# kai-neumann/OrthoSfM

Measured on AMD Instinct MI355X. Metric: image-pairs matched/sec + BA iterations/sec (N images, M tracks) at 1/2/4/8 GPU, higher is better.
Workload: dtype i8; 1 GPU; 50 orthographic images, 20000 SIFT features/img, exhaustive matching (1225 pairs, low-res gate + two-way + cross-check + lists; SURVEY 8d's unit of work: up to, not including, RANSAC-F -- the pass through RANSAC-F is `with_geometric_verification`); views=50, features_per_view=20000, pairs=1225

## Files before the change

### orthosfm_amd/csrc/match_api.hip

```cpp
#include <algorithm>
#include <atomic>
#include <cfloat>
#include <cmath>
#include <cstring>
#include <chrono>
#include <condition_variable>
#include <deque>
#include <functional>
#include <mutex>
#include <queue>
#include <thread>
#include <vector>

#include "match_kernels.h"
#include "cashash_kernels.h"
#include <random>
#include "osfm_common.h"
#include "ransac_kernels.h"

namespace osfm {

static thread_local std::string g_last_error;

void set_error(const char *fmt, ...)
{
    char buf[1024];
    va_list ap;
    va_start(ap, fmt);
    vsnprintf(buf, sizeof(buf), fmt, ap);
    va_end(ap);
    g_last_error = buf;
}

namespace {

inline int round_up(int x, int m) { return (x + m - 1) / m * m; }

struct ViewData {
    bool set = false;
    int ns = 0, nu = 0;
    int ns_pad = 0, nu_pad = 0;
    DeviceBuffer sift, sift_corr, surf, surf_corr;
    DeviceBuffer sift_raw, sift_raw_corr, special, special_corr, special_map, special_slot;
    int n_special = 0;
    int surf_norm2_max = 0;
    DeviceBuffer cas_hash[2], cas_bucket[2], cas_start[2], cas_items[2], cas_rec[2];
    DeviceBuffer positions;
    int n_positions = -1;
    hipEvent_t ready = nullptr;
    ~ViewData() { event_destroy(ready); }
    ViewData() = default;
    ViewData(const ViewData &) = delete;
    ViewData &operator=(const ViewData &) = delete;
};

void build_lowe_table(float lowe, bool is_signed, std::vector<int32_t> *tab)
{
    const volatile float sq = lowe * lowe;
    const float sq_lowe = sq;
    const int dmax = is_signed ? 32258 : 65534;
    tab->assign(32768, 0x7fffffff);
    for (int d2 = 0; d2 <= dmax; d2 += 2) {
        int lo = 0, hi = dmax / 2 + 1;
        while (lo < hi) {
            const int mid = (lo + hi) / 2;
            const float ratio = static_cast<float>(2 * mid) / static_cast<float>(d2);
            if (ratio > sq_lowe) hi = mid; else lo = mid + 1;
        }
        (*tab)[d2 / 2] = lo > dmax / 2 ? 0x7fffffff : 2 * lo;
    }
}

int max_d1_for(float dist_thres, bool is_signed)
{
    const volatile float sq = dist_thres * dist_thres;
    const float sq_dist = sq;
    const int dmax = is_signed ? 32258 : 65534;
    int best = -1;
    int lo = 0, hi = dmax;
    if (!(static_cast<float>(0) > sq_dist)) {
        while (lo < hi) {
            const int mid = (lo + hi + 1) / 2;
            if (static_cast<float>(mid) > sq_dist) hi = mid - 1; else lo = mid;
        }
        best = lo;
    }
    return best;
}

}
}

using namespace osfm;

struct osfm_matcher {
    int device = 0;
    hipStream_t stream = nullptr;
    osfm_match_options opts;
    std::vector<ViewData> views;
    DeviceBuffer lowe_sift, lowe_surf;
    LoweTable tab_sift, tab_surf;
    std::mutex mu;
    hipStream_t up_stream = nullptr;
    std::mutex up_mu;

    DeviceBuffer d_problems[2], rowparts, colparts, out, keep, mark_off[2], counts[2];
    DeviceBuffer exact_items, exact_count, stage_in, flags;
    DeviceBuffer sp_parts, sp_col, d_spjobs;
    DeviceBuffer clock_probe;
    DeviceBuffer zero_tile;
    int special_max = 512;
    int expect_pairs = 0;
    DeviceBuffer d_m12_off, d_len12, d_corr_off, d_keep_pair, d_corr;
    DeviceBuffer d_corr_alt;
    hipStream_t copy_stream = nullptr;
    hipEvent_t ev_compact[2] = {nullptr, nullptr}, ev_copied[2] = {nullptr, nullptr};
    bool copied_used[2] = {false, false};
    DeviceBuffer d_jobs, d_inl, d_inl_count, d_corr2, d_gather_off;
    hipEvent_t ev[2][2] = {{nullptr, nullptr}, {nullptr, nullptr}};
    hipEvent_t ev_sp[2] = {nullptr, nullptr};
    char *pin_ptr[2] = {nullptr, nullptr};
    size_t pin_bytes[2] = {0, 0};
    hipEvent_t pin_ev[2] = {nullptr, nullptr};
    bool pin_used[2] = {false, false};
    unsigned pin_next = 0;

    DeviceBuffer cas_proj[2], cas_sum[2], cas_avg[2], cas_state;
    std::atomic<bool> cas_dirty{true};

    osfm_match_stats stats;

    struct Staging { int32_t *ptr = nullptr; size_t ints = 0; int users = 0; };
    struct PairRequest {
        int kind;
        int v1, v2, num_features;
        int32_t *m12, *m21, *len12, *len21, *count;
        int status = OSFM_OK;
        bool done = false;
        std::string error;
        Staging *stage = nullptr;
        int64_t src12 = 0, src21 = 0;
        int32_t n12 = 0, n21 = 0;
    };
    std::vector<Staging *> comb_staging;

    std::vector<osfm_matcher *> shards;
    std::vector<Staging> shard_stage;
    std::atomic<unsigned> next_shard{0};
    std::mutex multi_mu;
    std::mutex comb_mu;
    std::condition_variable comb_cv;
    std::deque<PairRequest *> comb_queue;
    bool comb_leader = false;
};

namespace {

struct PairPlan {
    int v1, v2;
    int ns1, nu1, ns2, nu2;
    bool has_sift, has_surf;
    int64_t off12, off21;
    int len12, len21;
    int prob_index[2];
};

struct BatchResult {
    std::vector<PairPlan> plans;
    std::vector<int32_t> counts;
    int64_t out_ints = 0;
};

int check_view(const osfm_matcher *m, int v, const char *what)
{
    if (v < 0 || v >= (int)m->views.size()) {
        set_error("%s: view id %d out of range [0, %zu)", what, v, m->views.size());
        return OSFM_E_ARG;
    }
    if (!m->views[v].set) {
        set_error("%s: view %d has not been set", what, v);
        return OSFM_E_STATE;
    }
    return OSFM_OK;
}

struct BatchMode {
    int limit = 0;
    bool lowres = false;
    bool apply = true;
    int type_mask = 3;
    int expect = 0;
};

int ensure_cashash(osfm_matcher *m);

int run_batch(osfm_matcher *m, const osfm_pair *pairs, int num_pairs, const BatchMode &mode,
    BatchResult *res)
{
    const int lowres_limit = mode.limit;
    const bool cascade = m->opts.matcher_type == OSFM_MATCHER_CASCADE_HASHING && mode.limit == 0;
    if (cascade) OSFM_RETURN_IF(ensure_cashash(m));
    res->plans.assign(num_pairs, PairPlan());
    res->counts.assign(num_pairs, 0);
    std::vector<MatchProblem> probs[2];
    std::vector<SpecialJob> spjobs, spjobs_wide;
    struct SpEntry { int problem, side, view, units, nchunk; };
    std::vector<SpEntry> spentries;
    int64_t sp_recs = 0, sp_cols = 0;
    std::vector<int64_t> mark_off[2];
    int64_t out_ints = 0, rowpart_recs = 0, colpart_recs = 0, keep_bytes = 0, total_queries = 0;
    int total_blocks[2] = {0, 0}, max_n[2] = {0, 0};
    bool needs_mask[2] = {false, false};
    bool any_special[2] = {false, false};
    bool any_c0[2] = {false, false}, any_corrected[2] = {false, false};
    int64_t macs = 0, alg_bytes = 0, macs_surf = 0;
    int64_t cas_queries[2] = {0, 0};

    int64_t rb_estimate = 0;
    for (int p = 0; p < num_pairs; ++p) {
        const int v1 = pairs[p].view_1;
        if (v1 >= 0 && v1 < (int)m->views.size())
            rb_estimate += (std::max(m->views[v1].ns, m->views[v1].nu) + kRowsPerBlock - 1) / kRowsPerBlock;
    }
    static const int forced_seg_tiles = [] { const char *e = getenv("OSFM_SEG_TILES"); return e ? atoi(e) : 0; }();
    auto choose_seg_cols = [&](int n2) {
        const int ncyc = (n2 + kCycleCols - 1) / kCycleCols;
        int cyc;
        if (forced_seg_tiles > 0) cyc = std::max(1, forced_seg_tiles / 16);
        else {
            constexpr int64_t kWantBlocks = 2048;
            const int64_t want = (kWantBlocks + std::max<int64_t>(rb_estimate, 1) - 1) / std::max<int64_t>(rb_estimate, 1);
            const int nseg = (int)std::min<int64_t>(std::max<int64_t>(want, 1), ncyc);
            cyc = (ncyc + nseg - 1) / nseg;
        }
        cyc = std::min(cyc, kSegColsMax / kCycleCols);
        return cyc * kCycleCols;
    };

    for (int p = 0; p < num_pairs; ++p) {
        PairPlan &pl = res->plans[p];
        pl.v1 = pairs[p].view_1; pl.v2 = pairs[p].view_2;
        OSFM_RETURN_IF(check_view(m, pl.v1, "match"));
        OSFM_RETURN_IF(check_view(m, pl.v2, "match"));
        const ViewData &a = m->views[pl.v1], &b = m->views[pl.v2];
        pl.ns1 = a.ns; pl.nu1 = a.nu; pl.ns2 = b.ns; pl.nu2 = b.nu;
        pl.has_sift = a.ns > 0 && (mode.type_mask & 1);
        pl.has_surf = a.nu > 0 && (mode.type_mask & 2);
        if (cascade && !m->opts.cascade_keep_empty_blocks) {
            if (b.ns == 0) pl.has_sift = false;
            if (b.nu == 0) pl.has_surf = false;
        }
        if (mode.lowres && pl.has_sift) pl.has_surf = false;
        if (lowres_limit > 0) {
            pl.ns1 = std::min(pl.ns1, lowres_limit); pl.ns2 = std::min(pl.ns2, lowres_limit);
            pl.nu1 = std::min(pl.nu1, lowres_limit); pl.nu2 = std::min(pl.nu2, lowres_limit);
        }
        const int e1 = pl.has_sift ? pl.ns1 : 0;
        const int e2 = pl.has_sift ? pl.ns2 : 0;
        pl.len12 = e1 + (pl.has_surf ? pl.nu1 : 0);
        pl.len21 = e2 + (pl.has_surf ? pl.nu2 : 0);
        pl.off12 = out_ints; out_ints += round_up(pl.len12, 4);
        pl.off21 = out_ints; out_ints += round_up(pl.len21, 4);
        pl.prob_index[0] = pl.prob_index[1] = -1;
        for (int type = 0; type < 2; ++type) {
            if (type == 0 ? !pl.has_sift : !pl.has_surf) continue;
            MatchProblem pr;
            memset(&pr, 0, sizeof(pr));
            pr.n1 = type == 0 ? pl.ns1 : pl.nu1;
            pr.n2 = type == 0 ? pl.ns2 : pl.nu2;
            pr.A = (type == 0 ? a.sift : a.surf).as<int8_t>();
            pr.B = (type == 0 ? b.sift : b.surf).as<int8_t>();
            pr.corrA = (type == 0 ? a.sift_corr : a.surf_corr).as<int32_t>();
            pr.corrB = (type == 0 ? b.sift_corr : b.surf_corr).as<int32_t>();
            pr.A_raw = (type == 0 ? a.sift_raw : a.surf).as<int8_t>();
            pr.corrA_raw = (type == 0 ? a.sift_raw_corr : a.surf_corr).as<int32_t>();
            const bool limited = lowres_limit > 0;
            const int n_special = (type == 0 && !limited) ? a.n_special : 0;
            pr.n_special = n_special;
            pr.A_special = a.special.as<int8_t>();
            pr.corrA_special = a.special_corr.as<int32_t>();
            pr.special_map = a.special_map.as<int32_t>();
            pr.special_slot = n_special > 0 ? a.special_slot.as<int32_t>() : nullptr;
            const bool empty = pr.n1 == 0 || pr.n2 == 0;
            if (limited) needs_mask[type] = true;
            pr.B_raw = (type == 0 ? b.sift_raw : b.surf).as<int8_t>();
            pr.c0 = (type == 1 || b.n_special == 0) ? 1 : 0;
            if (type == 0 && !limited && !cascade && !empty && (a.n_special > 0 || b.n_special > 0) &&
                a.n_special <= m->special_max && b.n_special <= m->special_max) {
                pr.sp = 1; pr.c0 = 1;
                pr.nsA = a.n_special; pr.nsB = b.n_special;
                pr.n_special = 0;
                pr.special_slot = a.n_special > 0 ? a.special_slot.as<int32_t>() : nullptr;
                pr.B_special = b.special.as<int8_t>();
                pr.corrB_special = b.special_corr.as<int32_t>();
                pr.special_map_B = b.special_map.as<int32_t>();
                pr.special_slot_B = b.n_special > 0 ? b.special_slot.as<int32_t>() : nullptr;
                for (int side = 0; side < 2; ++side) {
                    const int ns = side == 0 ? pr.nsA : pr.nsB, no = side == 0 ? pr.n2 : pr.n1;
                    if (ns == 0) continue;
                    const int units = (ns + 31) / 32;
                    pr.sp_wide[side] = units > kSpSlots ? 1 : 0;
                    const int chunk_cols = pr.sp_wide[side] ? kSpWideChunk : kSpChunk;
                    const int nchunk = (no + chunk_cols - 1) / chunk_cols;
                    pr.sp_row_off[side] = sp_recs; sp_recs += (int64_t)nchunk * round_up(ns, 32);
                    pr.sp_col_off[side] = sp_cols; sp_cols += round_up(no, 32);
                    spentries.push_back({(int)probs[type].size(), side, side == 0 ? pl.v2 : pl.v1, units, nchunk});
                }
            }
            if (!empty && !limited) (pr.c0 ? any_c0 : any_corrected)[type] = true;
            if (!empty && pr.n_special > 0) any_special[type] = true;
            pr.nrb_main = empty ? 0 : (pr.n1 + kRowsPerBlock - 1) / kRowsPerBlock;
            pr.nrb = pr.nrb_main + (empty ? 0 : (pr.n_special + kRowsPerBlock - 1) / kRowsPerBlock);
            pr.seg_cols = (pr.c0 && !limited && pr.n_special == 0 && !empty) ? choose_seg_cols(pr.n2) : kSegCols;
            pr.nseg = empty ? 0 : (pr.n2 + pr.seg_cols - 1) / pr.seg_cols;
            pr.n2stride = round_up(pr.n2, kCycleCols);
            pr.block_start = total_blocks[type];
            if (cascade) {
                const ViewData *vd[2] = {&a, &b};
                for (int side = 0; side < 2; ++side) {
                    pr.cas_rec[side] = vd[side]->cas_rec[type].ptr;
                    pr.cas_start[side] = vd[side]->cas_start[type].as<int32_t>();
                    pr.cas_items[side] = vd[side]->cas_items[type].as<int32_t>();
                }
                pr.cas_state_off[0] = cas_queries[type]; cas_queries[type] += pr.n1;
                pr.cas_state_off[1] = cas_queries[type]; cas_queries[type] += pr.n2;
            } else {
                total_blocks[type] += pr.nrb * pr.nseg;
                pr.rowpart_off = rowpart_recs;
                rowpart_recs += (int64_t)pr.nseg * pr.nrb * kRowsPerBlock;
                pr.colpart_off = colpart_recs;
                colpart_recs += (int64_t)pr.nrb * pr.n2stride;
            }
            pr.m12 = reinterpret_cast<int32_t *>(pl.off12 + (type == 0 ? 0 : e1));
            pr.m21 = reinterpret_cast<int32_t *>(pl.off21 + (type == 0 ? 0 : e2));
            pr.out_off12 = (type == 1 && mode.apply) ? e2 : 0;
            pr.out_off21 = (type == 1 && mode.apply) ? e1 : 0;
            if (type == 1) {
                const long long bound = (long long)a.surf_norm2_max * (long long)b.surf_norm2_max;
                pr.force_exact = bound > 32767LL * 32767LL ? 1 : 0;
            }
            pl.prob_index[type] = (int)probs[type].size();
            mark_off[type].push_back(keep_bytes); keep_bytes += round_up(pr.n1, 16);
            mark_off[type].push_back(keep_bytes); keep_bytes += round_up(pr.n2, 16);
            max_n[type] = std::max(max_n[type], std::max(pr.n1, pr.n2));
            total_queries += pr.n1 + pr.n2;
            probs[type].push_back(pr);
            if (!empty) {
                const int dim = type == 0 ? 128 : 64;
                macs += (int64_t)pr.n1 * pr.n2 * dim;
                if (type == 1) macs_surf += (int64_t)pr.n1 * pr.n2 * dim;
                alg_bytes += (int64_t)(pr.n1 + pr.n2) * (dim + 4);
            }
        }
    }
    res->out_ints = out_ints;

    double grow = 1.0;
    if (mode.expect > num_pairs && num_pairs > 0) grow = 1.02 * (double)mode.expect / num_pairs;
    auto grown = [&](int64_t n) { return (size_t)((double)std::max<int64_t>(n, 1) * std::max(grow, 1.0)); };
    OSFM_RETURN_IF(m->out.reserve(grown(std::max<int64_t>(out_ints, 4)) * 4));
    OSFM_RETURN_IF(m->rowparts.reserve(grown(rowpart_recs) * sizeof(RowPart)));
    OSFM_RETURN_IF(m->colparts.reserve(grown(colpart_recs) * sizeof(ColPart)));
    OSFM_RETURN_IF(m->keep.reserve(grown(std::max<int64_t>(keep_bytes, 16))));
    OSFM_RETURN_IF(m->exact_items.reserve(grown(total_queries) * sizeof(ExactItem)));
    OSFM_RETURN_IF(m->exact_count.reserve(16));
    OSFM_RETURN_IF(m->sp_parts.reserve((size_t)std::max<int64_t>(sp_recs, 1) * sizeof(RowPart)));
    hipStream_t s = m->stream;
    {
        std::vector<uint8_t> seen(m->views.size(), 0);
        for (int p = 0; p < num_pairs; ++p)
            for (int v : {res->plans[p].v1, res->plans[p].v2})
                if (!seen[v]) { seen[v] = 1; if (m->views[v].ready) OSFM_HIP_CHECK(hipStreamWaitEvent(s, m->views[v].ready, 0)); }
    }
    std::stable_sort(spentries.begin(), spentries.end(), [](const SpEntry &x, const SpEntry &y) {
        return x.view != y.view ? x.view < y.view : x.units < y.units;
    });
    for (size_t e = 0; e < spentries.size();) {
        SpecialJob j;
        memset(&j, 0, sizeof(j));
        const SpEntry &f = spentries[e];
        if (f.units > kSpSlots) {
            j.problem[0] = f.problem; j.side[0] = f.side; j.count = 0;
            for (int c = 0; c < f.nchunk; ++c) { j.chunk = c; spjobs_wide.push_back(j); }
            ++e;
            continue;
        }
        if (f.units > 1) {
            j.problem[0] = f.problem; j.side[0] = f.side; j.count = 0;
            ++e;
        } else {
            int c = 0;
            while (c < kSpSlots && e < spentries.size() && spentries[e].view == f.view && spentries[e].units == 1) {
                j.problem[c] = spentries[e].problem; j.side[c] = spentries[e].side; ++c; ++e;
            }
            j.count = c;
        }
        for (int c = 0; c < f.nchunk; ++c) { j.chunk = c; spjobs.push_back(j); }
    }
    OSFM_RETURN_IF(m->sp_col.reserve((size_t)std::max<int64_t>(sp_cols, 1) * 4));
    OSFM_RETURN_IF(m->d_spjobs.reserve(std::max<size_t>(spjobs.size() + spjobs_wide.size(), 1) * sizeof(SpecialJob)));
    if (!spjobs.empty())
        OSFM_HIP_CHECK(hipMemcpyAsync(m->d_spjobs.ptr, spjobs.data(), spjobs.size() * sizeof(SpecialJob),
            hipMemcpyHostToDevice, s));
    if (!spjobs_wide.empty())
        OSFM_HIP_CHECK(hipMemcpyAsync(m->d_spjobs.as<SpecialJob>() + spjobs.size(), spjobs_wide.data(),
            spjobs_wide.size() * sizeof(SpecialJob), hipMemcpyHostToDevice, s));
    int32_t *d_out = m->out.as<int32_t>();
    OSFM_HIP_CHECK(hipMemsetAsync(d_out, 0xff, (size_t)std::max<int64_t>(out_ints, 4) * 4, s));

    OSFM_HIP_CHECK(hipMemsetAsync(m->exact_count.ptr, 0, 16, s));
    bool timed[2] = {false, false};
    bool probed = false;
    for (int type = 0; type < 2; ++type) {
        const int np = (int)probs[type].size();
        if (np == 0) continue;
        for (auto &pr : probs[type]) {
            pr.m12 = d_out + reinterpret_cast<intptr_t>(pr.m12);
            pr.m21 = d_out + reinterpret_cast<intptr_t>(pr.m21);
        }
        OSFM_RETURN_IF(m->d_problems[type].reserve(np * sizeof(MatchProblem)));
        OSFM_RETURN_IF(m->mark_off[type].reserve(np * 2 * sizeof(int64_t)));
        OSFM_RETURN_IF(m->counts[type].reserve(np * sizeof(int32_t)));
        OSFM_HIP_CHECK(hipMemcpyAsync(m->d_problems[type].ptr, probs[type].data(),
            np * sizeof(MatchProblem), hipMemcpyHostToDevice, s));
        OSFM_HIP_CHECK(hipMemcpyAsync(m->mark_off[type].ptr, mark_off[type].data(),
            np * 2 * sizeof(int64_t), hipMemcpyHostToDevice, s));
        OSFM_HIP_CHECK(hipMemsetAsync(m->counts[type].ptr, 0, np * sizeof(int32_t), s));
        const MatchProblem *dp = m->d_problems[type].as<MatchProblem>();
        const LoweTable tab = type == 0 ? m->tab_sift : m->tab_surf;
        const int ecap = (int)std::min<int64_t>(total_queries, 0x7fffffff);
        int32_t *ecount = m->exact_count.as<int32_t>() + type;

        if (cascade) {
            OSFM_HIP_CHECK(hipEventRecord(m->ev[type][0], s));
            timed[type] = true;
            OSFM_RETURN_IF(m->cas_state.reserve((size_t)std::max<int64_t>(cas_queries[type], 1) * kCasMaxCand * 4));
            launch_cashash_match(type == 0 ? 128 : 64, dp, np, max_n[type], m->cas_state.as<int32_t>(), tab, s);
            OSFM_HIP_CHECK(hipEventRecord(m->ev[type][1], s));
        } else {
            if (total_blocks[type] > 0) { OSFM_HIP_CHECK(hipEventRecord(m->ev[type][0], s)); timed[type] = true; }
            unsigned long long *probe = nullptr;
            if (type == 0 && mode.limit == 0) {
                OSFM_RETURN_IF(m->clock_probe.reserve(16));
                OSFM_HIP_CHECK(hipMemsetAsync(m->clock_probe.ptr, 0, 16, s));
                probe = m->clock_probe.as<unsigned long long>();
                probed = true;
            }
            if (!m->zero_tile.ptr) {
                OSFM_RETURN_IF(m->zero_tile.reserve((size_t)kTileCols * 128));
                OSFM_HIP_CHECK(hipMemsetAsync(m->zero_tile.ptr, 0, (size_t)kTileCols * 128, s));
            }
            launch_match_tiles(type == 0 ? 8 : 4, needs_mask[type], any_special[type], any_c0[type],
                any_corrected[type], dp, np, total_blocks[type],
                m->rowparts.as<RowPart>(), m->colparts.as<ColPart>(), s, probe, m->zero_tile.as<int8_t>());
            if (timed[type]) OSFM_HIP_CHECK(hipEventRecord(m->ev[type][1], s));
            if (type == 0 && !(spjobs.empty() && spjobs_wide.empty())) {
                OSFM_HIP_CHECK(hipEventRecord(m->ev_sp[0], s));
                launch_match_special(dp, m->d_spjobs.as<SpecialJob>(), (int)spjobs.size(), m->sp_parts.as<RowPart>(),
                    m->sp_col.as<int32_t>(), s);
                launch_match_special_wide(dp, m->d_spjobs.as<SpecialJob>() + spjobs.size(), (int)spjobs_wide.size(),
                    m->sp_parts.as<RowPart>(), m->sp_col.as<int32_t>(), s);
                OSFM_HIP_CHECK(hipEventRecord(m->ev_sp[1], s));
            }
            launch_match_finish(dp, np, max_n[type], m->rowparts.as<RowPart>(),
                m->colparts.as<ColPart>(), m->sp_parts.as<RowPart>(), m->sp_col.as<int32_t>(), tab, 0,
                m->exact_items.as<ExactItem>(), ecount, ecap, s);
            launch_exact_scan(type == 0 ? 128 : 64, dp, m->exact_items.as<ExactItem>(), ecount, ecap,
                tab, s);
        }
        launch_cross_check_mark(dp, np, max_n[type], m->keep.as<uint8_t>(), m->keep.as<uint8_t>(),
            m->mark_off[type].as<int64_t>(), m->counts[type].as<int32_t>(), s);
        if (mode.apply)
            launch_cross_check_apply(dp, np, max_n[type], m->keep.as<uint8_t>(),
                m->keep.as<uint8_t>(), m->mark_off[type].as<int64_t>(), s);
        OSFM_HIP_CHECK(hipGetLastError());
    }

    std::vector<int32_t> hc[2];
    int32_t hexact[4] = {0, 0, 0, 0};
    for (int type = 0; type < 2; ++type) {
        hc[type].resize(probs[type].size());
        if (!hc[type].empty())
            OSFM_HIP_CHECK(hipMemcpyAsync(hc[type].data(), m->counts[type].ptr,
                hc[type].size() * sizeof(int32_t), hipMemcpyDeviceToHost, s));
    }
    OSFM_HIP_CHECK(hipMemcpyAsync(hexact, m->exact_count.ptr, 16, hipMemcpyDeviceToHost, s));
    unsigned long long hprobe[2] = {0, 0};
    if (probed) OSFM_HIP_CHECK(hipMemcpyAsync(hprobe, m->clock_probe.ptr, 16, hipMemcpyDeviceToHost, s));
    OSFM_HIP_CHECK(hipStreamSynchronize(s));
    m->stats.tile_shader_cycles += (double)hprobe[0];
    m->stats.tile_refclk_ticks += (double)hprobe[1];
    for (int p = 0; p < num_pairs; ++p) {
        int c = 0;
        for (int type = 0; type < 2; ++type)
            if (res->plans[p].prob_index[type] >= 0) c += hc[type][res->plans[p].prob_index[type]];
        res->counts[p] = c;
    }
    for (int type = 0; type < 2; ++type) {
        if (!timed[type]) continue;
        float ms = 0.f;
        OSFM_HIP_CHECK(hipEventElapsedTime(&ms, m->ev[type][0], m->ev[type][1]));
        if (cascade) {
            m->stats.cashash_kernel_ms += ms;
            m->stats.cashash_kernel_launches += 1;
        } else if (mode.limit > 0) {
            m->stats.lowres_kernel_ms += ms;
            m->stats.lowres_kernel_launches += 1;
        } else {
            m->stats.tile_kernel_ms += ms;
            m->stats.tile_kernel_launches += 1;
            if (type == 1) { m->stats.surf_tile_kernel_ms += ms; m->stats.surf_tile_kernel_launches += 1; }
        }
    }
    if (!(spjobs.empty() && spjobs_wide.empty())) {
        float ms = 0.f;
        OSFM_HIP_CHECK(hipEventElapsedTime(&ms, m->ev_sp[0], m->ev_sp[1]));
        m->stats.special_kernel_ms += ms;
        m->stats.special_kernel_launches += 1;
    }
    m->stats.exact_scan_queries += hexact[0] + hexact[1];
    if (cascade) {
    } else if (mode.limit > 0) {
        m->stats.lowres_mac_count += macs;
    } else {
        m->stats.mac_count += macs;
        m->stats.surf_mac_count += macs_surf;
        m->stats.algorithmic_bytes += alg_bytes;
    }
    return OSFM_OK;
}

int upload_view(osfm_matcher *m, int view, const uint16_t *sift, int n_sift, const int16_t *surf,
    int n_surf)
{
    if (view < 0 || view >= (int)m->views.size()) {
        set_error("set_view: view id %d out of range", view);
        return OSFM_E_ARG;
    }
    if (n_sift < 0 || n_surf < 0 || (n_sift > 0 && !sift) || (n_surf > 0 && !surf)) {
        set_error("set_view: null descriptors / negative count");
        return OSFM_E_ARG;
    }
    ViewData &v = m->views[view];
    hipStream_t s = m->up_stream;
    v.set = false;
    v.ns = n_sift; v.nu = n_surf;
    v.ns_pad = round_up(std::max(n_sift, 1), kRowsPerBlock);
    v.nu_pad = round_up(std::max(n_surf, 1), kRowsPerBlock);
    OSFM_RETURN_IF(v.sift.reserve((size_t)v.ns_pad * 128));
// ... 1174 lines not shown
```

### orthosfm_amd/csrc/match_kernels.h

```cpp
#pragma once
#include <hip/hip_runtime.h>
#include <stdint.h>

namespace osfm {

constexpr int kRowsPerBlock = 256;
constexpr int kTileCols = 64;
constexpr int kSegCols = 8192;
constexpr int kSegColsMax = 32768;
constexpr int kCycleCols = 1024;
constexpr int kKeyNone = -(1 << 30);

struct MatchProblem {
    const int8_t *A;
    const int8_t *B;
    const int32_t *corrA;
    const int32_t *corrB;
    int32_t n1, n2;
    int32_t nrb, nseg;
    int32_t n2stride;
    int32_t seg_cols;
    int32_t block_start;
    int64_t rowpart_off;
    int64_t colpart_off;
    int32_t *m12;
    int32_t *m21;
    int32_t out_off12;
    int32_t out_off21;
    int32_t force_exact;
    int32_t nrb_main;
    const int8_t *A_raw;
    const int32_t *corrA_raw;
    const int8_t *A_special;
    const int32_t *corrA_special;
    const int32_t *special_map;
    const int32_t *special_slot;
    int32_t n_special;
    int32_t c0;
    const int8_t *B_raw;
    int32_t sp;
    int32_t nsA, nsB;
    const int8_t *B_special;
    const int32_t *corrB_special;
    const int32_t *special_map_B;
    const int32_t *special_slot_B;
    int64_t sp_row_off[2];
    int64_t sp_col_off[2];
    int32_t sp_wide[2];
    const void *cas_rec[2];
    const int32_t *cas_start[2];
    const int32_t *cas_items[2];
    int64_t cas_state_off[2];
};

struct RowPart { int32_t ip_best, idx_best, ip_second, pad; };
struct ColPart { int32_t key_best, key_second; };

__device__ __forceinline__ int xcd_remap(int bid, int total)
{
    const int q = total >> 3, r = total & 7;
    const int xcd = bid & 7, slot = bid >> 3;
    const int base = xcd < r ? xcd * (q + 1) : r * (q + 1) + (xcd - r) * q;
    return base + slot;
}

struct LoweTable {
    const int32_t *reject_from;
    int32_t max_d1;
    int32_t is_signed;
};

struct ExactItem { int32_t problem; int32_t dir; int32_t query; };

constexpr int kSpChunk = 4096;
constexpr int kSpSlots = 2;
struct SpecialJob { int32_t problem[4], side[4]; int32_t count, chunk, pad0, pad1; };
void launch_match_special(const MatchProblem *d_problems, const SpecialJob *d_jobs, int num_jobs,
    RowPart *sp_parts, int32_t *sp_col, hipStream_t s);
constexpr int kSpWideChunk = 1024;
constexpr int kSpWideUnits = 8;
void launch_match_special_wide(const MatchProblem *d_problems, const SpecialJob *d_jobs, int num_jobs,
    RowPart *sp_parts, int32_t *sp_col, hipStream_t s);

void launch_match_tiles(int ch, bool masked, bool any_special, bool any_c0, bool any_corrected,
    const MatchProblem *d_problems,
    int num_problems, int total_blocks, RowPart *rowparts, ColPart *colparts, hipStream_t s,
    unsigned long long *clock_probe = nullptr,
    const int8_t *zero_tile = nullptr);

void launch_match_finish(const MatchProblem *d_problems, int num_problems,
    int max_n, const RowPart *rowparts, const ColPart *colparts, const RowPart *sp_parts, const int32_t *sp_col, LoweTable tab,
    int force_exact, ExactItem *exact_items, int32_t *exact_count, int exact_cap,
    hipStream_t s);

void launch_exact_scan(int dim, const MatchProblem *d_problems,
    const ExactItem *items, const int32_t *count, int exact_cap, LoweTable tab,
    hipStream_t s);

void launch_cross_check_mark(const MatchProblem *d_problems, int num_problems, int max_n,
    uint8_t *keep12, uint8_t *keep21, const int64_t *mark_off, int32_t *counts, hipStream_t s);
void launch_cross_check_apply(const MatchProblem *d_problems, int num_problems, int max_n,
    const uint8_t *keep12, const uint8_t *keep21, const int64_t *mark_off, hipStream_t s);

void launch_compact_pairs(int num_pairs, const int32_t *m12_all, const int64_t *m12_off,
    const int32_t *len12, const int64_t *corr_off, const uint8_t *keep, int32_t *corr,
    hipStream_t s);

void launch_gather_inliers(int num, const int32_t *corr, const int32_t *inl, const int64_t *src_off,
    const int64_t *dst_off, const int32_t *counts, int32_t *out, hipStream_t s);

void launch_prepare_sift(const uint16_t *src, int n, int npad, int8_t *dst,
    int32_t *corr, int8_t *dst_raw, int32_t *corr_raw, int32_t *range_err, hipStream_t s);
void launch_gather_rows(const int8_t *src, const int32_t *corr, const int32_t *map, int n, int npad,
    int dim, int32_t pad_corr, int8_t pad_byte, int8_t *dst, int32_t *dst_corr, hipStream_t s);
void launch_prepare_surf(const int16_t *src, int n, int npad, int8_t *dst,
    int32_t *corr, int32_t *norm2max, int32_t *range_err, hipStream_t s);

}
```

### orthosfm_amd/csrc/match_kernels.hip

```cpp
#include <algorithm>

#include "match_kernels.h"

namespace osfm {


typedef int v4i __attribute__((ext_vector_type(4)));
typedef int v16i __attribute__((ext_vector_type(16)));


__device__ __forceinline__ int max3i(int a, int b, int c)
{
    int r;
    asm("v_max3_i32 %0, %1, %2, %3" : "=v"(r) : "v"(a), "v"(b), "v"(c));
    return r;
}
__device__ __forceinline__ int med3a(int a, int b, int c)
{
    int r;
    asm("v_med3_i32 %0, %1, %2, %3" : "=v"(r) : "v"(a), "v"(b), "v"(c));
    return r;
}

constexpr int kGroupTiles = 8;
// ... 550 lines not shown
                cand[u][j] = sidx < pd.n_special ? pd.special_map[sidx] : -1;
            }
        }
    }
#pragma unroll
    for (int u = 0; u < 2; ++u) {
#pragma unroll
        for (int j = 0; j < J; ++j) {
            const int cs = max(cand[u][j], 0);
            cv[u][j] = *reinterpret_cast<const int4 *>(Cm + (size_t)cs * DIM + c * 16);
            corr_c[u][j] = corrC[cs];
        }
    }
#pragma unroll
    for (int u = 0; u < 2; ++u) {
        int kbest = INT_MIN, ksec = INT_MIN;
#pragma unroll
        for (int j = 0; j < J; ++j) {
            int acc = __builtin_amdgcn_sdot4(qv[u].x, cv[u][j].x, 0, false);
            acc = __builtin_amdgcn_sdot4(qv[u].y, cv[u][j].y, acc, false);
            acc = __builtin_amdgcn_sdot4(qv[u].z, cv[u][j].z, acc, false);
            acc = __builtin_amdgcn_sdot4(qv[u].w, cv[u][j].w, acc, false);
            acc += dpp_mov<kDppXor1>(acc, 0);
            acc += dpp_mov<kDppXor2>(acc, 0);
            if (LPC == 8) acc += dpp_mov<kDppHalfMirror>(acc, 0);
            const int key = cand[u][j] >= 0 ? (acc + corr_q[u] + corr_c[u][j]) * 32 + (j * CPL + k) : INT_MIN;
            ksec = med3a(kbest, ksec, key);
            kbest = max(kbest, key);
        }
        const int wbest = wave_max(kbest);
        const int wsec = wave_max(kbest == wbest ? ksec : kbest);
        const int pos = wbest & 31;
        int widx = 0;
#pragma unroll
        for (int j = 0; j < J; ++j)
            if ((pos / CPL) == j) widx = __builtin_amdgcn_readlane(cand[u][j], (pos % CPL) * LPC);
        idx_out[u] = max(widx, 0);
        best_out[u] = wbest >> 5;
        second_out[u] = wsec == INT_MIN ? INT_MIN : wsec >> 5;
    }
}

template <int DIM>
__device__ __forceinline__ void
scan_specials(const MatchProblem &pd, int dir, int q, int lane, int &best_out, int &second_out, int &idx_out)
{
    constexpr int LPC = DIM / 16, CPL = 64 / LPC;
    const int c = lane % LPC, k = lane / LPC;
    const int8_t *Q = dir == 0 ? pd.A : pd.B;
    const int8_t *Cm = dir == 0 ? pd.B_special : pd.A_special;
    const int32_t *corrC = dir == 0 ? pd.corrB_special : pd.corrA_special;
    const int32_t *map = dir == 0 ? pd.special_map_B : pd.special_map;
    const int ns = dir == 0 ? pd.nsB : pd.nsA;
    const int4 qv = *reinterpret_cast<const int4 *>(Q + (size_t)q * DIM + c * 16);
    const int corr_q = (dir == 0 ? pd.corrA : pd.corrB)[q];
    int kbest = INT_MIN, ksec = INT_MIN;
    for (int base = 0; base < ns; base += CPL) {
        const int slot = base + k;
        const bool live = slot < ns;
        const int4 cv = *reinterpret_cast<const int4 *>(Cm + (size_t)(live ? slot : 0) * DIM + c * 16);
        int acc = __builtin_amdgcn_sdot4(qv.x, cv.x, 0, false);
        acc = __builtin_amdgcn_sdot4(qv.y, cv.y, acc, false);
        acc = __builtin_amdgcn_sdot4(qv.z, cv.z, acc, false);
        acc = __builtin_amdgcn_sdot4(qv.w, cv.w, acc, false);
        acc += dpp_mov<kDppXor1>(acc, 0);
        acc += dpp_mov<kDppXor2>(acc, 0);
        if (LPC == 8) acc += dpp_mov<kDppHalfMirror>(acc, 0);
        const int key = live ? (acc + corr_q + corrC[live ? slot : 0]) * 512 + slot : INT_MIN;
        ksec = med3a(kbest, ksec, key);
        kbest = max(kbest, key);
    }
    const int wbest = wave_max(kbest);
    const int wsec = wave_max(kbest == wbest ? ksec : kbest);
    best_out = wbest >> 9;
    second_out = wsec == INT_MIN ? INT_MIN : wsec >> 9;
    idx_out = map[wbest & 511];
}

template <int DIM, bool SIGNED>
__global__ __launch_bounds__(128) void
match_finish_kernel(const MatchProblem *__restrict__ problems, const RowPart *__restrict__ rowparts,
    const ColPart *__restrict__ colparts, const RowPart *__restrict__ sp_parts, const int32_t *__restrict__ sp_col,
    LoweTable tab, int force_exact, ExactItem *__restrict__ exact_items, int32_t *__restrict__ exact_count, int exact_cap,
    int blocks_per_dir, int total_blocks)
{
    const int lin = xcd_remap(blockIdx.x, total_blocks);
    const int problem = lin / (2 * blocks_per_dir), within = lin - problem * 2 * blocks_per_dir;
    const MatchProblem &pd = problems[problem];
    const int dir = within / blocks_per_dir;
    const int block_x = within - dir * blocks_per_dir;
    const int q = block_x * blockDim.x + threadIdx.x;
    const int lane = threadIdx.x & 63;
    const int nq = dir == 0 ? pd.n1 : pd.n2;
    const int nc = dir == 0 ? pd.n2 : pd.n1;
    if ((int)(block_x * blockDim.x) >= nq) return;
    int32_t *out = dir == 0 ? pd.m12 : pd.m21;
    const bool active = q < nq;

    int ip1 = INT_MIN, ip2 = INT_MIN, idx1 = 0, code = 0, kind1 = 0;
    int sp_slot = -1;
    if (active && nc > 0 && pd.sp) {
        const int ns_mine = dir == 0 ? pd.nsA : pd.nsB;
        if (ns_mine > 0) sp_slot = (dir == 0 ? pd.special_slot : pd.special_slot_B)[q];
        if (sp_slot >= 0) {
            const int ns_pad = (ns_mine + 31) & ~31;
            const int chunk_cols = pd.sp_wide[dir] ? kSpWideChunk : kSpChunk;
            const int nchunk = (nc + chunk_cols - 1) / chunk_cols;
            const RowPart *rp0 = sp_parts + pd.sp_row_off[dir] + sp_slot;
            for (int c = 0; c < nchunk; ++c) {
                const RowPart p = rp0[(int64_t)c * ns_pad];
                ip2 = max(max(ip2, p.ip_second), min(ip1, p.ip_best));
                if (p.ip_best >= ip1 && p.ip_best != INT_MIN) { ip1 = p.ip_best; idx1 = p.idx_best; }
            }
            kind1 = pd.sp_wide[dir] ? 4 : 3;
        }
    }
    bool sp_scan = false;
    int sp_m1 = INT_MIN;
    if (active && nc > 0 && sp_slot < 0) {
        if (dir == 0) {
            const int64_t stride = (int64_t)pd.nrb * kRowsPerBlock;
            int slot = q;
            if (pd.special_slot && !pd.sp) {
                const int sidx = pd.special_slot[q];
                if (sidx >= 0) slot = pd.nrb_main * kRowsPerBlock + sidx;
            }
            constexpr int kBatch = 4;
            const RowPart *rp0 = rowparts + pd.rowpart_off + slot;
            const int nseg = pd.nseg;
            for (int s0 = 0; s0 < nseg; s0 += kBatch) {
                RowPart p[kBatch];
#pragma unroll
                for (int u = 0; u < kBatch; ++u) p[u] = rp0[(int64_t)min(s0 + u, nseg - 1) * stride];
                __builtin_amdgcn_sched_barrier(0);
#pragma unroll
                for (int u = 0; u < kBatch; ++u) {
                    const bool live = s0 + u < nseg;
                    const int pb = live ? p[u].ip_best : INT_MIN, ps = live ? p[u].ip_second : INT_MIN;
                    ip2 = max(max(ip2, ps), min(ip1, pb));
                    if (pb >= ip1 && pb != INT_MIN) { ip1 = pb; idx1 = p[u].idx_best; kind1 = p[u].pad; }
                }
            }
        } else {
            constexpr int kBatch = 8;
            const ColPart *cp0 = colparts + pd.colpart_off + q;
            const int nrb = pd.nrb;
            const int64_t stride = pd.n2stride;
            for (int rb0 = 0; rb0 < nrb; rb0 += kBatch) {
                ColPart p[kBatch];
#pragma unroll
                for (int u = 0; u < kBatch; ++u)
                {
                    const unsigned long long raw = __builtin_nontemporal_load(
                        reinterpret_cast<const unsigned long long *>(cp0 + (int64_t)min(rb0 + u, nrb - 1) * stride));
                    p[u].key_best = (int)(raw & 0xffffffffu); p[u].key_second = (int)(raw >> 32);
                }
                __builtin_amdgcn_sched_barrier(0);
#pragma unroll
                for (int u = 0; u < kBatch; ++u) {
                    const bool live = rb0 + u < nrb;
                    const int pb = (!live || p[u].key_best == kKeyNone) ? INT_MIN : (p[u].key_best >> 8);
                    const int ps = (!live || p[u].key_second == kKeyNone) ? INT_MIN : (p[u].key_second >> 8);
                    ip2 = max(max(ip2, ps), min(ip1, pb));
                    if (pb >= ip1 && pb != INT_MIN) { ip1 = pb; idx1 = rb0 + u; code = p[u].key_best & 255; }
                }
            }
        }
        if (pd.sp && (dir == 0 ? pd.nsB : pd.nsA) > 0) {
            const int t1 = sp_col[pd.sp_col_off[dir ^ 1] + q];
            if (t1 >= ip1 && t1 != INT_MIN) {
                sp_m1 = ip1; ip1 = t1; sp_scan = true;
            } else {
                ip2 = max(ip2, t1);
            }
        }
    }
    const int limit = tab.is_signed ? 32767 : 65535;
    bool exact = active && nc > 0 && (force_exact || pd.force_exact || ip1 > limit);
    bool refine = false;
    int res = -1;
    if (active && nc > 0 && !exact) {
        res = accept_match(ip1, sp_scan ? max(sp_m1, ip2) : ip2, 0, tab);
        if (res >= 0) {
            if (ip1 < 0) { res = 0; sp_scan = false; }
            else if ((sp_scan ? sp_m1 : ip2) == ip1) { exact = true; sp_scan = false; }
            else if (!sp_scan) refine = true;
        } else {
            sp_scan = false;
        }
    } else {
        sp_scan = false;
    }
    unsigned long long todo = __ballot(refine);
    int rbest = 0, rsecond = 0, ridx = 0;
    while (todo) {
        int src[2], qs[2], is[2], cs[2], ks[2], idx[2], found[2], second[2];
        src[0] = __ffsll((long long)todo) - 1;
        todo &= todo - 1;
        src[1] = todo ? __ffsll((long long)todo) - 1 : src[0];
        todo &= todo - 1;
#pragma unroll
        for (int u = 0; u < 2; ++u) {
            qs[u] = __builtin_amdgcn_readlane(q, src[u]);
            is[u] = __builtin_amdgcn_readlane(idx1, src[u]);
            cs[u] = __builtin_amdgcn_readlane(code, src[u]);
            ks[u] = __builtin_amdgcn_readlane(kind1, src[u]);
        }
        if (dir == 0) rescan_groups<DIM, 0>(pd, qs, is, cs, ks, lane, idx, found, second);
        else rescan_groups<DIM, 1>(pd, qs, is, cs, ks, lane, idx, found, second);
#pragma unroll
        for (int u = 0; u < 2; ++u)
            if (lane == src[u]) { rbest = found[u]; rsecond = second[u]; ridx = idx[u]; }
    }
    if (refine) {
        rsecond = max(rsecond, ip2);
        res = accept_match(rbest, rsecond, ridx, tab);
        if (res >= 0 && rsecond == rbest) exact = true;
    }
    unsigned long long todo2 = __ballot(sp_scan);
    while (todo2) {
        const int src = __ffsll((long long)todo2) - 1;
        todo2 &= todo2 - 1;
        const int qs = __builtin_amdgcn_readlane(q, src);
        int wb, ws, wi;
        scan_specials<DIM>(pd, dir, qs, lane, wb, ws, wi);
        if (lane == src) { rbest = wb; rsecond = ws; ridx = wi; }
    }
    if (sp_scan) {
        rsecond = max(max(rsecond, sp_m1), ip2);
        res = accept_match(rbest, rsecond, ridx, tab);
        if (res >= 0 && rsecond == rbest) exact = true;
    }
    if (exact) {
        const int slot = atomicAdd(exact_count, 1);
        if (slot < exact_cap) {
            ExactItem it;
            it.problem = problem; it.dir = dir; it.query = q;
            exact_items[slot] = it;
        }
    }
    if (active) out[q] = res;
}

void launch_match_finish(const MatchProblem *d_problems, int num_problems, int max_n,
    const RowPart *rowparts, const ColPart *colparts, const RowPart *sp_parts, const int32_t *sp_col, LoweTable tab, int force_exact,
    ExactItem *exact_items, int32_t *exact_count, int exact_cap, hipStream_t s)
{
    if (num_problems <= 0 || max_n <= 0) return;
    const int blocks_per_dir = (max_n + 127) / 128;
    const int64_t total = (int64_t)blocks_per_dir * 2 * num_problems;
    if (total > INT_MAX) return;
    const dim3 grid((unsigned)total);
    if (tab.is_signed)
        hipLaunchKernelGGL((match_finish_kernel<64, true>), grid, dim3(128), 0, s, d_problems, rowparts,
            colparts, sp_parts, sp_col, tab, force_exact, exact_items, exact_count, exact_cap, blocks_per_dir, (int)total);
    else
        hipLaunchKernelGGL((match_finish_kernel<128, false>), grid, dim3(128), 0, s, d_problems, rowparts,
            colparts, sp_parts, sp_col, tab, force_exact, exact_items, exact_count, exact_cap, blocks_per_dir, (int)total);
}

template <int DIM, bool SIGNED>
__global__ __launch_bounds__(256) void
exact_scan_kernel(const MatchProblem *__restrict__ problems, const ExactItem *__restrict__ items,
    const int32_t *__restrict__ count, int exact_cap, LoweTable tab)
{
    const int lane = threadIdx.x & 63;
    const int wave_global = (blockIdx.x * blockDim.x + threadIdx.x) >> 6;
    const int nwaves = (gridDim.x * blockDim.x) >> 6;
    const int n_items = min(*count, exact_cap);
    for (int it = wave_global; it < n_items; it += nwaves) {
        const ExactItem item = items[it];
        const MatchProblem &pd = problems[item.problem];
        const int8_t *Q = item.dir == 0 ? pd.A : pd.B;
        const int8_t *C = item.dir == 0 ? pd.B : pd.A;
        const int nc = item.dir == 0 ? pd.n2 : pd.n1;
        int32_t *out = item.dir == 0 ? pd.m12 : pd.m21;
        const int8_t *qrow = Q + (size_t)item.query * DIM;
        int best = 0, second = 0, idx = 0;
        for (int base = 0; base < nc; base += 64) {
            const int j = base + lane;
            int ip = 0;
            if (j < nc) {
                const int8_t *crow = C + (size_t)j * DIM;
                unsigned lanes[8] = {0, 0, 0, 0, 0, 0, 0, 0};
                for (int k = 0; k < DIM; k += 8) {
#pragma unroll
                    for (int l = 0; l < 8; ++l) {
                        const int qa = SIGNED ? (int)qrow[k + l] : (int)qrow[k + l] + 128;
                        const int ca = SIGNED ? (int)crow[k + l] : (int)crow[k + l] + 128;
                        lanes[l] += (unsigned)(qa * ca);
                    }
                }
#pragma unroll
                for (int l = 0; l < 8; ++l)
                    ip += SIGNED ? (int)(short)(lanes[l] & 0xffffu) : (int)(lanes[l] & 0xffffu);
            }
            const int cnt = min(64, nc - base);
            for (int l = 0; l < cnt; ++l) {
                const int v = __shfl(ip, l);
                if (v >= second) {
                    if (v >= best) {
                        second = best;
                        best = SIGNED ? (int)(short)v : (int)(unsigned short)v;
                        idx = base + l;
                    } else {
                        second = SIGNED ? (int)(short)v : (int)(unsigned short)v;
                    }
                }
            }
        }
        if (lane == 0) {
            int d1, d2;
            if (SIGNED) {
                const int b = min(16129, max(0, best)), s2 = min(16129, max(0, second));
                d1 = (int)(short)(32258 - 2 * b); d2 = (int)(short)(32258 - 2 * s2);
            } else {
                const int b = min(65025, best), s2 = min(65025, second);
                d1 = min(32767, 65025 - b) * 2; d2 = min(32767, 65025 - s2) * 2;
            }
            int res = idx;
            if (d1 > tab.max_d1) res = -1;
            else if (d1 >= tab.reject_from[d2 >> 1]) res = -1;
            out[item.query] = res;
        }
    }
}

void launch_exact_scan(int dim, const MatchProblem *d_problems, const ExactItem *items,
    const int32_t *count, int exact_cap, LoweTable tab, hipStream_t s)
{
    if (exact_cap <= 0) return;
    const dim3 grid(1024), block(256);
    if (dim == 128)
        hipLaunchKernelGGL((exact_scan_kernel<128, false>), grid, block, 0, s, d_problems, items,
            count, exact_cap, tab);
    else
        hipLaunchKernelGGL((exact_scan_kernel<64, true>), grid, block, 0, s, d_problems, items,
            count, exact_cap, tab);
}

constexpr int kCheckPerThread = 8;
// ... 243 lines not shown
```

Before: 23220 pairs/s.

## Defer finish-kernel refine rescans into bucketed MFMA rescore kernel

Instead of each wave in the finish kernel serially rescanning candidate groups for queries that need refinement, such queries are appended to per-strip or per-window buckets via atomics. A new rescore kernel then batches the queries of each bucket and recomputes their dot products against the bucket's shared candidate set with int8 MFMA, applying the correction terms and the Lowe test. This removes divergent per-query rescans at the cost of an extra launch, a memset, atomics and item buffers. Queries that overflow a bucket still take the old rescan path.

```diff
diff --git a/orthosfm_amd/csrc/match_api.hip b/orthosfm_amd/csrc/match_api.hip
--- a/orthosfm_amd/csrc/match_api.hip
+++ b/orthosfm_amd/csrc/match_api.hip
@@ -106,6 +106,7 @@
 
     DeviceBuffer d_problems[2], rowparts, colparts, out, keep, mark_off[2], counts[2];
     DeviceBuffer exact_items, exact_count, stage_in, flags;
+    DeviceBuffer rs_count, rs_items;
     DeviceBuffer sp_parts, sp_col, d_spjobs;
     DeviceBuffer clock_probe;
     DeviceBuffer zero_tile;
@@ -215,6 +216,7 @@
     bool any_c0[2] = {false, false}, any_corrected[2] = {false, false};
     int64_t macs = 0, alg_bytes = 0, macs_surf = 0;
     int64_t cas_queries[2] = {0, 0};
+    int64_t rs_buckets = 0, rs_items = 0;
 
     int64_t rb_estimate = 0;
     for (int p = 0; p < num_pairs; ++p) {
@@ -315,6 +317,12 @@
             pr.nseg = empty ? 0 : (pr.n2 + pr.seg_cols - 1) / pr.seg_cols;
             pr.n2stride = round_up(pr.n2, kCycleCols);
             pr.block_start = total_blocks[type];
+            pr.rs_bucket_off = rs_buckets;
+            pr.rs_item_off = rs_items;
+            if (type == 0 && !cascade && !empty) {
+                rs_buckets += rescore_buckets(pr.nrb_main, pr.n2);
+                rs_items += rescore_items(pr.nrb_main, pr.n2);
+            }
             if (cascade) {
                 const ViewData *vd[2] = {&a, &b};
                 for (int side = 0; side < 2; ++side) {
@@ -364,6 +372,13 @@
     OSFM_RETURN_IF(m->keep.reserve(grown(std::max<int64_t>(keep_bytes, 16))));
     OSFM_RETURN_IF(m->exact_items.reserve(grown(total_queries) * sizeof(ExactItem)));
     OSFM_RETURN_IF(m->exact_count.reserve(16));
+    const char *rescan_env = getenv("OSFM_FINISH_RESCAN");
+    const bool bucketed = rs_buckets > 0 && rs_buckets <= INT_MAX && max_n[0] < (1 << 26) &&
+                          !(rescan_env && strcmp(rescan_env, "wave") == 0);
+    if (bucketed) {
+        OSFM_RETURN_IF(m->rs_count.reserve(grown(rs_buckets) * sizeof(int32_t)));
+        OSFM_RETURN_IF(m->rs_items.reserve(grown(rs_items) * sizeof(RescoreItem)));
+    }
     OSFM_RETURN_IF(m->sp_parts.reserve((size_t)std::max<int64_t>(sp_recs, 1) * sizeof(RowPart)));
     hipStream_t s = m->stream;
     {
@@ -462,9 +477,15 @@
                     m->sp_parts.as<RowPart>(), m->sp_col.as<int32_t>(), s);
                 OSFM_HIP_CHECK(hipEventRecord(m->ev_sp[1], s));
             }
+            const bool rs = type == 0 && bucketed;
+            if (rs) OSFM_HIP_CHECK(hipMemsetAsync(m->rs_count.ptr, 0, (size_t)rs_buckets * sizeof(int32_t), s));
             launch_match_finish(dp, np, max_n[type], m->rowparts.as<RowPart>(),
                 m->colparts.as<ColPart>(), m->sp_parts.as<RowPart>(), m->sp_col.as<int32_t>(), tab, 0,
-                m->exact_items.as<ExactItem>(), ecount, ecap, s);
+                m->exact_items.as<ExactItem>(), ecount, ecap, rs ? m->rs_count.as<int32_t>() : nullptr,
+                rs ? m->rs_items.as<RescoreItem>() : nullptr, s);
+            if (rs)
+                launch_match_rescore(dp, np, m->rs_count.as<int32_t>(), m->rs_items.as<RescoreItem>(), rs_buckets, tab,
+                    m->exact_items.as<ExactItem>(), ecount, ecap, s);
             launch_exact_scan(type == 0 ? 128 : 64, dp, m->exact_items.as<ExactItem>(), ecount, ecap,
                 tab, s);
         }
diff --git a/orthosfm_amd/csrc/match_kernels.h b/orthosfm_amd/csrc/match_kernels.h
--- a/orthosfm_amd/csrc/match_kernels.h
+++ b/orthosfm_amd/csrc/match_kernels.h
@@ -51,6 +51,8 @@
     const int32_t *cas_start[2];
     const int32_t *cas_items[2];
     int64_t cas_state_off[2];
+    int64_t rs_bucket_off;
+    int64_t rs_item_off;
 };
 
 struct RowPart { int32_t ip_best, idx_best, ip_second, pad; };
@@ -88,10 +90,23 @@
     unsigned long long *clock_probe = nullptr,
     const int8_t *zero_tile = nullptr);
 
+constexpr int kRescoreWin = 17;
+constexpr int kRescoreCap0 = 32, kRescoreCap1 = 64;
+struct RescoreItem { int32_t q_sub; int32_t ip2; };
+__host__ __device__ inline int rescore_windows(int n2) { return ((n2 + kTileCols - 1) / kTileCols + kRescoreWin - 1) / kRescoreWin; }
+__host__ __device__ inline int rescore_buckets(int nrb_main, int n2) { return nrb_main * 4 + 32 * rescore_windows(n2); }
+__host__ __device__ inline int64_t rescore_items(int nrb_main, int n2)
+{
+    return (int64_t)nrb_main * 4 * kRescoreCap1 + (int64_t)32 * rescore_windows(n2) * kRescoreCap0;
+}
+
 void launch_match_finish(const MatchProblem *d_problems, int num_problems,
     int max_n, const RowPart *rowparts, const ColPart *colparts, const RowPart *sp_parts, const int32_t *sp_col, LoweTable tab,
     int force_exact, ExactItem *exact_items, int32_t *exact_count, int exact_cap,
-    hipStream_t s);
+    int32_t *rs_count, RescoreItem *rs_items, hipStream_t s);
+void launch_match_rescore(const MatchProblem *d_problems, int num_problems, const int32_t *rs_count,
+    const RescoreItem *rs_items, int64_t total_buckets, LoweTable tab, ExactItem *exact_items, int32_t *exact_count,
+    int exact_cap, hipStream_t s);
 
 void launch_exact_scan(int dim, const MatchProblem *d_problems,
     const ExactItem *items, const int32_t *count, int exact_cap, LoweTable tab,
diff --git a/orthosfm_amd/csrc/match_kernels.hip b/orthosfm_amd/csrc/match_kernels.hip
--- a/orthosfm_amd/csrc/match_kernels.hip
+++ b/orthosfm_amd/csrc/match_kernels.hip
@@ -656,7 +656,7 @@
 match_finish_kernel(const MatchProblem *__restrict__ problems, const RowPart *__restrict__ rowparts,
     const ColPart *__restrict__ colparts, const RowPart *__restrict__ sp_parts, const int32_t *__restrict__ sp_col,
     LoweTable tab, int force_exact, ExactItem *__restrict__ exact_items, int32_t *__restrict__ exact_count, int exact_cap,
-    int blocks_per_dir, int total_blocks)
+    int32_t *__restrict__ rs_count, RescoreItem *__restrict__ rs_items, int blocks_per_dir, int total_blocks)
 {
     const int lin = xcd_remap(blockIdx.x, total_blocks);
     const int problem = lin / (2 * blocks_per_dir), within = lin - problem * 2 * blocks_per_dir;
@@ -765,6 +765,34 @@
     } else {
         sp_scan = false;
     }
+    bool deferred = false;
+    if (!SIGNED && DIM == 128 && rs_count != nullptr && refine) {
+        int b = -1, sub = 0, cap = 0;
+        int64_t item = 0;
+        const int nb1 = pd.nrb_main * 4;
+        if (dir == 1) {
+            if (kind1 == 0 && idx1 < pd.nrb_main && code < 8) {
+                b = idx1 * 4 + (code >> 1); sub = code & 1;
+                item = (int64_t)b * kRescoreCap1; cap = kRescoreCap1;
+            }
+        } else if (kind1 == 1) {
+            const int tq = idx1 >> 6;
+            if (tq < (pd.n2 + kTileCols - 1) / kTileCols) {
+                const int w = tq / kRescoreWin, k = w * 32 + (idx1 & 31);
+                b = nb1 + k; sub = tq - w * kRescoreWin;
+                item = (int64_t)nb1 * kRescoreCap1 + (int64_t)k * kRescoreCap0; cap = kRescoreCap0;
+            }
+        }
+        if (b >= 0) {
+            const int slot = atomicAdd(rs_count + pd.rs_bucket_off + b, 1);
+            if (slot < cap) {
+                RescoreItem it;
+                it.q_sub = q * 32 + sub; it.ip2 = ip2;
+                rs_items[pd.rs_item_off + item + slot] = it;
+                refine = false; deferred = true;
+            }
+        }
+    }
     unsigned long long todo = __ballot(refine);
     int rbest = 0, rsecond = 0, ridx = 0;
     while (todo) {
@@ -813,12 +841,12 @@
             exact_items[slot] = it;
         }
     }
-    if (active) out[q] = res;
+    if (active && !deferred) out[q] = res;
 }
 
 void launch_match_finish(const MatchProblem *d_problems, int num_problems, int max_n,
     const RowPart *rowparts, const ColPart *colparts, const RowPart *sp_parts, const int32_t *sp_col, LoweTable tab, int force_exact,
-    ExactItem *exact_items, int32_t *exact_count, int exact_cap, hipStream_t s)
+    ExactItem *exact_items, int32_t *exact_count, int exact_cap, int32_t *rs_count, RescoreItem *rs_items, hipStream_t s)
 {
     if (num_problems <= 0 || max_n <= 0) return;
     const int blocks_per_dir = (max_n + 127) / 128;
@@ -827,10 +855,168 @@
     const dim3 grid((unsigned)total);
     if (tab.is_signed)
         hipLaunchKernelGGL((match_finish_kernel<64, true>), grid, dim3(128), 0, s, d_problems, rowparts,
-            colparts, sp_parts, sp_col, tab, force_exact, exact_items, exact_count, exact_cap, blocks_per_dir, (int)total);
+            colparts, sp_parts, sp_col, tab, force_exact, exact_items, exact_count, exact_cap, nullptr, nullptr,
+            blocks_per_dir, (int)total);
     else
         hipLaunchKernelGGL((match_finish_kernel<128, false>), grid, dim3(128), 0, s, d_problems, rowparts,
-            colparts, sp_parts, sp_col, tab, force_exact, exact_items, exact_count, exact_cap, blocks_per_dir, (int)total);
+            colparts, sp_parts, sp_col, tab, force_exact, exact_items, exact_count, exact_cap, rs_count, rs_items,
+            blocks_per_dir, (int)total);
+}
+
+constexpr int kRescorePerWave = 16;
+static_assert(2 * (kRescoreWin + 15) <= 64, "a direction-0 bucket's candidates fill two MFMA blocks at most");
+
+__global__ __launch_bounds__(256, 4) void
+match_rescore_kernel(const MatchProblem *__restrict__ problems, int num_problems, const int32_t *__restrict__ rs_count,
+    const RescoreItem *__restrict__ rs_items, int total_buckets, int total_blocks, LoweTable tab,
+    ExactItem *__restrict__ exact_items, int32_t *__restrict__ exact_count, int exact_cap)
+{
+    __shared__ __attribute__((aligned(16))) int corr_s[4][64];
+    const int lin = xcd_remap(blockIdx.x, total_blocks);
+    const int wv = threadIdx.x >> 6, lane = threadIdx.x & 63, h = lane >> 5, j = lane & 31;
+    const int b0 = (lin * 4 + wv) * kRescorePerWave;
+    if (b0 >= total_buckets) return;
+    const int cnt_l = lane < kRescorePerWave && b0 + lane < total_buckets ? rs_count[b0 + lane] : 0;
+    unsigned long long todo = __ballot(cnt_l > 0);
+    if (!todo) return;
+    int p = 0;
+    {
+        const int b = b0 + __ffsll((long long)todo) - 1;
+        int lo = 0, hi = num_problems - 1;
+        while (lo < hi) {
+            const int mid = (lo + hi + 1) >> 1;
+            if (problems[mid].rs_bucket_off <= b) lo = mid; else hi = mid - 1;
+        }
+        p = lo;
+    }
+    const v16i zero16 = {0, 0, 0, 0, 0, 0, 0, 0, 0, 0, 0, 0, 0, 0, 0, 0};
+    while (todo) {
+        const int k = __ffsll((long long)todo) - 1;
+        todo &= todo - 1;
+        const int b = b0 + k;
+        while (p + 1 < num_problems && problems[p + 1].rs_bucket_off <= b) ++p;
+        const MatchProblem &pd = problems[p];
+        const int local = b - (int)pd.rs_bucket_off;
+        const int nb1 = pd.nrb_main * 4;
+        const int dir = local < nb1 ? 1 : 0;
+        int strip = 0, w0 = 0, lr = 0, cap;
+        int64_t item0;
+        if (dir == 1) {
+            strip = (local >> 2) * kRowsPerBlock + (local & 3) * 64;
+            cap = kRescoreCap1;
+            item0 = pd.rs_item_off + (int64_t)local * kRescoreCap1;
+        } else {
+            const int l0 = local - nb1;
+            w0 = (l0 >> 5) * kRescoreWin; lr = l0 & 31;
+            cap = kRescoreCap0;
+            item0 = pd.rs_item_off + (int64_t)nb1 * kRescoreCap1 + (int64_t)l0 * kRescoreCap0;
+        }
+        auto cand_of = [&](int o) {
+            if (dir == 1) { const int r = strip + o; return r < pd.n1 ? r : -1; }
+            const int c = kTileCols * (w0 + (o >> 1)) + 32 * (o & 1) + lr;
+            return c < pd.n2 ? c : -1;
+        };
+        const int cnt = min(__builtin_amdgcn_readlane(cnt_l, k), cap);
+        const int8_t *Cm = dir == 0 ? pd.B : pd.A;
+        const int8_t *Qm = dir == 0 ? pd.A : pd.B;
+        const int32_t *corrC = dir == 0 ? pd.corrB : pd.corrA;
+        const int32_t *corrQ = dir == 0 ? pd.corrA : pd.corrB;
+        int32_t *out = dir == 0 ? pd.m12 : pd.m21;
+        RescoreItem it0;
+        it0.q_sub = 0; it0.ip2 = 0;
+        if (j < cnt) it0 = rs_items[item0 + j];
+        v4i a[2][4];
+#pragma unroll
+        for (int bk = 0; bk < 2; ++bk) {
+            const int cs = max(cand_of(32 * bk + j), 0);
+#pragma unroll
+            for (int ks = 0; ks < 4; ++ks)
+                a[bk][ks] = *reinterpret_cast<const v4i *>(Cm + (size_t)cs * 128 + (ks * 2 + h) * 16);
+        }
+        {
+            const int c = cand_of(lane);
+            corr_s[wv][lane] = c >= 0 ? corrC[c] : INT_MIN;
+        }
+        __builtin_amdgcn_wave_barrier();
+        for (int qb = 0; qb < cnt; qb += 32) {
+            const bool live = qb + j < cnt;
+            RescoreItem it = it0;
+            if (qb > 0) {
+                it.q_sub = 0; it.ip2 = 0;
+                if (live) it = rs_items[item0 + qb + j];
+            }
+            const int q = it.q_sub >> 5, sub = it.q_sub & 31;
+            v4i bq[4];
+#pragma unroll
+            for (int ks = 0; ks < 4; ++ks)
+                bq[ks] = *reinterpret_cast<const v4i *>(Qm + (size_t)q * 128 + (ks * 2 + h) * 16);
+            const int cq = corrQ[q];
+            v16i acc[2];
+#pragma unroll
+            for (int bk = 0; bk < 2; ++bk) {
+                acc[bk] = __builtin_amdgcn_mfma_i32_32x32x32_i8(a[bk][0], bq[0], zero16, 0, 0, 0);
+#pragma unroll
+                for (int ks = 1; ks < 4; ++ks)
+                    acc[bk] = __builtin_amdgcn_mfma_i32_32x32x32_i8(a[bk][ks], bq[ks], acc[bk], 0, 0, 0);
+            }
+            int kbest = INT_MIN, ksec = INT_MIN;
+#pragma unroll
+            for (int bk = 0; bk < 2; ++bk)
+#pragma unroll
+                for (int g = 0; g < 4; ++g) {
+                    const int ob = 32 * bk + 8 * g + 4 * h;
+                    const v4i cc = *reinterpret_cast<const v4i *>(&corr_s[wv][ob]);
+#pragma unroll
+                    for (int e = 0; e < 4; ++e) {
+                        const int o = ob + e;
+                        int n;
+                        bool ok;
+                        if (dir == 1) {
+                            n = 16 * bk + 4 * g + e;
+                            ok = h == sub;
+                        } else {
+                            n = o - 2 * sub;
+                            ok = (unsigned)n < 32u;
+                        }
+                        const int key = ok && cc[e] != INT_MIN ? (acc[bk][4 * g + e] + cq + cc[e]) * 32 + n : INT_MIN;
+                        ksec = med3a(kbest, ksec, key);
+                        kbest = max(kbest, key);
+                    }
+                }
+            const int obest = __shfl_xor(kbest, 32), osec = __shfl_xor(ksec, 32);
+            const int wbest = max(kbest, obest);
+            const int wsec = max(min(kbest, obest), max(ksec, osec));
+            if (live && h == 0) {
+                const int pos = wbest & 31;
+                const int o = dir == 1 ? 32 * (pos >> 4) + (pos & 3) + 8 * ((pos >> 2) & 3) + 4 * sub : pos + 2 * sub;
+                const int idx = max(cand_of(o), 0);
+                const int rbest = wbest >> 5;
+                const int rsecond = max(wsec == INT_MIN ? INT_MIN : wsec >> 5, it.ip2);
+                const int res = accept_match(rbest, rsecond, idx, tab);
+                out[q] = res;
+                if (res >= 0 && rsecond == rbest) {
+                    const int slot = atomicAdd(exact_count, 1);
+                    if (slot < exact_cap) {
+                        ExactItem e;
+                        e.problem = p; e.dir = dir; e.query = q;
+                        exact_items[slot] = e;
+                    }
+                }
+            }
+        }
+        __builtin_amdgcn_wave_barrier();
+    }
+}
+
+void launch_match_rescore(const MatchProblem *d_problems, int num_problems, const int32_t *rs_count,
+    const RescoreItem *rs_items, int64_t total_buckets, LoweTable tab, ExactItem *exact_items, int32_t *exact_count,
+    int exact_cap, hipStream_t s)
+{
+    if (num_problems <= 0 || total_buckets <= 0) return;
+    const int64_t blocks = (total_buckets + 4 * kRescorePerWave - 1) / (4 * kRescorePerWave);
+    if (total_buckets > INT_MAX || blocks > INT_MAX) return;
+    hipLaunchKernelGGL(match_rescore_kernel, dim3((unsigned)blocks), dim3(256), 0, s, d_problems, num_problems,
+        rs_count, rs_items, (int)total_buckets, (int)blocks, tab, exact_items, exact_count, exact_cap);
 }
 
 template <int DIM, bool SIGNED>
```

Result: faster. 23610 pairs/s, median of 6 (+1.7%).
